# linwe2012/CourseComputationalPhotography

Measured on AMD Instinct MI355X. Metric: Gauss-Seidel pixel-updates/s on WxH 5-point Poisson grid, higher is better.
Workload: dtype f64

## Files before the change

### coursecomputationalphotography_amd/capi.py

```python
from __future__ import annotations

import atexit
import ctypes as C
import os
import sys
import weakref
from typing import Optional

import numpy as np

_HERE = os.path.dirname(os.path.abspath(__file__))
LIB_PATH = os.environ.get("CCP_GS_LIB") or os.path.join(_HERE, "lib", "libccp_gs.so")

CCP_OK = 0
GRID_DIRICHLET_MASK = 1
GRID_WEIGHTED = 2
MG_HIERARCHY_GALERKIN, MG_HIERARCHY_RESCALED = 0, 1
MG_HIERARCHIES = {"galerkin": MG_HIERARCHY_GALERKIN, "rescaled": MG_HIERARCHY_RESCALED}
ORDER_LEXICOGRAPHIC = 0
ORDER_MULTICOLOUR = 1
CLONE_IMPORT = 0
CLONE_MIXED = 1

ABI_SYMBOLS = (
    "ccp_status_string", "ccp_abi_version", "ccp_device_count",
    "ccp_csr_create", "ccp_csr_destroy", "ccp_csr_upload", "ccp_csr_upload_rows", "ccp_csr_rows_info", "ccp_csr_set_colouring", "ccp_csr_get_colouring", "ccp_csr_insert", "ccp_csr_insert_many", "ccp_csr_edit_stats", "ccp_csr_device_footprint", "ccp_csr_last_path", "ccp_csr_embed_region_host",
    "ccp_csr_gauss_seidel", "ccp_csr_conjugate_gradient", "ccp_csr_conjugate_gradient_jacobi", "ccp_csr_apply_to_vector", "ccp_csr_residual_norm2",
    "ccp_grid_create", "ccp_grid_destroy", "ccp_grid_get_layout", "ccp_grid_set_stream",
    "ccp_grid_synchronize", "ccp_grid_set_b_host", "ccp_grid_set_x_host", "ccp_grid_get_x_host",
    "ccp_grid_get_b_host", "ccp_grid_set_mask_host", "ccp_grid_fill_x", "ccp_grid_b_from_x", "ccp_grid_randomize_x",
    "ccp_grid_sweep", "ccp_grid_sweep_edges_first", "ccp_grid_stream_wait_edges", "ccp_grid_tune", "ccp_grid_set_fused", "ccp_grid_set_tiling", "ccp_grid_get_tiling", "ccp_grid_sweep_l1", "ccp_grid_halo_refreshed", "ccp_grid_gauss_seidel", "ccp_grid_gauss_seidel_lexicographic", "ccp_debug_lex_tickets", "ccp_grid_conjugate_gradient",
    "ccp_grid_mg_conjugate_gradient", "ccp_grid_mg_apply", "ccp_grid_mg_level",
    "ccp_grid_mg_set_hierarchy", "ccp_grid_mg_get_hierarchy",
    "ccp_grid_residual_norm2", "ccp_grid_abs_sum", "ccp_grid_assemble_rhs", "ccp_grid_assemble_from_images", "ccp_grid_store_u8",
    "ccp_grid_set_x_u8", "ccp_grid_assemble_region_rhs", "ccp_grid_assemble_clone", "ccp_grid_store_u8_composite",
    "ccp_grid_last_timing", "ccp_grid_region_begin", "ccp_grid_region_end",
    "ccp_grid_set_b_device", "ccp_grid_set_x_device", "ccp_grid_get_x_device", "ccp_grid_get_b_device",
    "ccp_grid_assemble_rhs_device", "ccp_grid_assemble_from_images_device", "ccp_grid_store_u8_device", "ccp_grid_set_x_u8_device",
    "ccp_grid_assemble_region_rhs_device", "ccp_grid_assemble_clone_device", "ccp_grid_store_u8_composite_device",
    "ccp_grid_set_weights_host", "ccp_grid_set_weights_device", "ccp_grid_assemble_weighted_rhs", "ccp_grid_assemble_weighted_rhs_device",
    "ccp_comm_probe", "ccp_comm_unique_id", "ccp_comm_create", "ccp_comm_destroy", "ccp_comm_info", "ccp_comm_all_reduce_sum", "ccp_comm_all_reduce_max",
    "ccp_grid_attach_comm", "ccp_grid_set_overlap", "ccp_grid_exchange_halos", "ccp_grid_sweep_rowblocked",
    "ccp_grid_gauss_seidel_rowblocked", "ccp_grid_conjugate_gradient_rowblocked", "ccp_grid_residual_norm2_global", "ccp_grid_comm_stats",
    "ccp_grid_mg_conjugate_gradient_rowblocked", "ccp_grid_mg_apply_rowblocked", "ccp_grid_mg_rowblock_info",
)


class CcpError(RuntimeError):
    def __init__(self, status: int, what: str):
        self.status = status
        super().__init__(f"{what}: status {status} ({status_string(status)})")


class Report(C.Structure):
    _fields_ = [("iterations", C.c_int32), ("converged", C.c_int32),
                ("last_l1_step", C.c_double), ("seconds", C.c_double)]


class GridDesc(C.Structure):
    _fields_ = [("width", C.c_int32), ("height", C.c_int32), ("channels", C.c_int32),
                ("row_begin", C.c_int32), ("row_count", C.c_int32), ("ghost", C.c_int32),
                ("device", C.c_int32), ("flags", C.c_int32)]


# ... 87 lines not shown
    L.ccp_csr_last_path.argtypes = [vp, C.POINTER(i32), C.POINTER(i32), C.POINTER(i32), C.POINTER(i64)]
    L.ccp_csr_edit_stats.argtypes = [vp] + [C.POINTER(i64)] * 5
    L.ccp_csr_device_footprint.argtypes = [vp] + [C.POINTER(i64)] * 2
    L.ccp_csr_gauss_seidel.argtypes = [vp, vp, vp, vp, dbl, i32, i32, i32, C.POINTER(Report)]
    L.ccp_csr_conjugate_gradient.argtypes = [vp, vp, vp, vp, dbl, i32, C.POINTER(Report)]
    L.ccp_csr_conjugate_gradient_jacobi.argtypes = [vp, vp, vp, dbl, i32, C.POINTER(Report)]
    L.ccp_grid_conjugate_gradient.argtypes = [vp, dbl, i32, C.POINTER(Report)]
    L.ccp_grid_mg_conjugate_gradient.argtypes = [vp, dbl, i32, i32, C.POINTER(Report)]
    L.ccp_grid_mg_apply.argtypes = [vp, i32]
    L.ccp_grid_mg_level.argtypes = [vp, i32] + [C.POINTER(i32)] * 3 + [vp] * 3
    L.ccp_grid_mg_set_hierarchy.argtypes = [vp, i32]
    L.ccp_grid_mg_get_hierarchy.argtypes = [vp, C.POINTER(i32)]
    L.ccp_csr_apply_to_vector.argtypes = [vp, vp, vp]
    L.ccp_csr_residual_norm2.argtypes = [vp, vp, vp, C.POINTER(dbl), C.POINTER(dbl)]
    L.ccp_grid_create.argtypes = [C.POINTER(GridDesc), C.POINTER(vp)]
    L.ccp_grid_destroy.argtypes = [vp]
    L.ccp_grid_get_layout.argtypes = [vp, C.POINTER(GridLayout)]
    L.ccp_grid_set_stream.argtypes = [vp, vp]
    L.ccp_grid_synchronize.argtypes = [vp]
    for name in ("ccp_grid_set_b_host", "ccp_grid_set_x_host", "ccp_grid_get_x_host", "ccp_grid_get_b_host"):
        getattr(L, name).argtypes = [vp, i32, vp, i32, i32]
    L.ccp_grid_set_mask_host.argtypes = [vp, vp, i64]
    L.ccp_grid_fill_x.argtypes = [vp, dbl]
    L.ccp_grid_b_from_x.argtypes = [vp]
    L.ccp_grid_randomize_x.argtypes = [vp, C.c_uint64, dbl, dbl]
    L.ccp_grid_sweep.argtypes = [vp, i32]
    L.ccp_grid_sweep_edges_first.argtypes = [vp, i32, i32]
    L.ccp_grid_stream_wait_edges.argtypes = [vp, vp]
    L.ccp_grid_sweep_l1.argtypes = [vp, vp]
    L.ccp_grid_tune.argtypes = [vp, i32, C.POINTER(i32), C.POINTER(i32), C.POINTER(C.c_float)]
    L.ccp_grid_set_fused.argtypes = [vp, i32]
    L.ccp_grid_set_tiling.argtypes = [vp, i32, i32]
    L.ccp_grid_get_tiling.argtypes = [vp, C.POINTER(i32), C.POINTER(i32), C.POINTER(i32)]
    L.ccp_grid_halo_refreshed.argtypes = [vp]
    L.ccp_grid_gauss_seidel.argtypes = [vp, dbl, i32, i32, C.POINTER(Report)]
    L.ccp_grid_gauss_seidel_lexicographic.argtypes = [vp, dbl, i32, i32, C.POINTER(Report)]
    L.ccp_grid_residual_norm2.argtypes = [vp, vp]
    L.ccp_grid_abs_sum.argtypes = [vp, vp]
    L.ccp_grid_assemble_rhs.argtypes = [vp, vp, vp, i64, vp]
    L.ccp_grid_assemble_from_images.argtypes = [vp, vp, i32, i64, vp, i64, i32]
    L.ccp_grid_store_u8.argtypes = [vp, vp, i64]
    L.ccp_grid_set_x_u8.argtypes = [vp, vp, i64]
    L.ccp_grid_assemble_region_rhs.argtypes = [vp, vp, vp, i64, vp, i64, i32]
    L.ccp_grid_assemble_clone.argtypes = [vp, vp, i64, vp, i64, i32, i32]
    L.ccp_grid_store_u8_composite.argtypes = [vp, vp, i64, vp, i64]
    da = C.POINTER(DeviceArray)
    for name in ("ccp_grid_set_b_device", "ccp_grid_set_x_device", "ccp_grid_get_x_device", "ccp_grid_get_b_device"):
        getattr(L, name).argtypes = [vp, da, i32, i32]
    L.ccp_grid_assemble_rhs_device.argtypes = [vp, da, da, vp]
    L.ccp_grid_assemble_from_images_device.argtypes = [vp, da, i32, da, i32]
    L.ccp_grid_store_u8_device.argtypes = [vp, da]
    L.ccp_grid_set_x_u8_device.argtypes = [vp, da]
    L.ccp_grid_assemble_region_rhs_device.argtypes = [vp, da, da, da, i32]
    L.ccp_grid_assemble_clone_device.argtypes = [vp, da, da, i32, i32]
    L.ccp_grid_store_u8_composite_device.argtypes = [vp, da, da]
    L.ccp_grid_set_weights_host.argtypes = [vp, vp, vp, vp, i64]
    L.ccp_grid_set_weights_device.argtypes = [vp, da, da, da]
    L.ccp_grid_assemble_weighted_rhs.argtypes = [vp, vp, vp, i64, vp, i64, i32]
    L.ccp_grid_assemble_weighted_rhs_device.argtypes = [vp, da, da, da, i32]
    L.ccp_grid_last_timing.argtypes = [vp, C.POINTER(C.c_float), C.POINTER(i32)]
    L.ccp_grid_region_begin.argtypes = [vp]
    L.ccp_grid_region_end.argtypes = [vp, C.POINTER(C.c_float), C.POINTER(i64), C.POINTER(i64)]
    L.ccp_comm_probe.argtypes = [i32]
    L.ccp_comm_unique_id.argtypes = [vp]
    L.ccp_comm_create.argtypes = [vp, i32, i32, i32, C.POINTER(vp)]
    L.ccp_comm_destroy.argtypes = [vp]
# ... 1 lines not shown
    L.ccp_comm_all_reduce_sum.argtypes = [vp, vp, i32]
    L.ccp_comm_all_reduce_max.argtypes = [vp, vp, i32]
    L.ccp_grid_attach_comm.argtypes = [vp, vp]
    L.ccp_grid_set_overlap.argtypes = [vp, i32]
    L.ccp_grid_exchange_halos.argtypes = [vp]
    L.ccp_grid_sweep_rowblocked.argtypes = [vp, i32]
    L.ccp_grid_gauss_seidel_rowblocked.argtypes = [vp, dbl, i32, i32, C.POINTER(Report)]
    L.ccp_grid_conjugate_gradient_rowblocked.argtypes = [vp, dbl, i32, C.POINTER(Report)]
    L.ccp_grid_mg_conjugate_gradient_rowblocked.argtypes = [vp, dbl, i32, i32, C.POINTER(Report)]
    L.ccp_grid_mg_apply_rowblocked.argtypes = [vp, i32]
    L.ccp_grid_mg_rowblock_info.argtypes = [vp] + [C.POINTER(i32)] * 4
    L.ccp_grid_residual_norm2_global.argtypes = [vp, vp]
    L.ccp_grid_comm_stats.argtypes = [vp, C.POINTER(i64), C.POINTER(i32), C.POINTER(i32), C.POINTER(i32)]
    _lib = L
    return L


def status_string(status: int) -> str:
    try:
        return load().ccp_status_string(status).decode()
    except Exception:
        return "?"


def check(status: int, what: str) -> None:
    if status != CCP_OK:
        raise CcpError(status, what)


def device_count() -> int:
    return int(load().ccp_device_count())


def _ptr(a: Optional[np.ndarray]):
    return None if a is None else a.ctypes.data_as(C.c_void_p)


def _f64(a) -> np.ndarray:
    return np.ascontiguousarray(a, dtype=np.float64)


def _i32(a) -> np.ndarray:
    return np.ascontiguousarray(a, dtype=np.int32)


def _no_overlap(shape, strides) -> bool:
    dims = sorted((s, e) for s, e in zip(strides, shape) if e > 1)
    span = 1
    for s, e in dims:
        if s < span:
            return False
        span = s * e
    return True


COMM_ID_BYTES = 128


def comm_probe(device: int = 0) -> None:
    _share_rccl_with_torch()
    check(load().ccp_comm_probe(device), "ccp_comm_probe")


def comm_unique_id() -> bytes:
    _share_rccl_with_torch()
    buf = (C.c_uint8 * COMM_ID_BYTES)()
# ... 681 lines not shown
```

### coursecomputationalphotography_amd/csrc/ccp_grid.hip

```cpp
#include "ccp_grid_kernels.hpp"
#include "ccp_grid_fused.hpp"
#include "ccp_grid_fused_wide.hpp"
#include "ccp_grid_lex.hpp"
#include "ccp_cg.hpp"
#include "ccp_grid_cg.hpp"
#include "ccp_grid_mg_view.hpp"
#include "ccp_grid_blend.hpp"
#include "ccp_grid_weighted.hpp"
#include "ccp_comm.hpp"

#include <algorithm>
#include <functional>
#include <cstring>
#include <chrono>
#include <vector>

using namespace ccp;

constexpr int kEdgeRing = 64;

struct ccp_grid {
    ccp_grid_desc desc{};
    Geom geom{};
    int ghost_top = 0, ghost_bottom = 0;
    bool shrink_top = false, shrink_bottom = false;
    int device = 0;
    hipStream_t stream = nullptr;
    hipStream_t stream2 = nullptr;
    hipEvent_t ev_main = nullptr, ev_side = nullptr;
    unsigned long long *edge_counter = nullptr;
    unsigned long long *edge_flag = nullptr;
    unsigned long long edge_epoch = 0;
    unsigned *edge_timeout = nullptr;
    unsigned long long edge_timeout_ticks = 200000000ull;
    int wait_mode = 0;
// ... 6 lines not shown
    hipEvent_t ev_comm = nullptr, ev_ready = nullptr;
    bool overlap = true;
    long exchanges = 0;
    DevBuf<double> x, b;
    DevBuf<double> cg_r, cg_p, cg_p2, cg_ap;
    DevBuf<CgState> cg_state;
    DevBuf<double> x_alt;
    bool allow_swap = false;
    bool masked = false;
    DevBuf<unsigned char> maskp, tile_live;
    DevBuf<int> tile_rows;
    DevBuf<unsigned char> mask_edge;
    bool mask_edge_known = false;
    int mask_border = -1;
    int live_T = -1, live_R = -1, live_lo = -1, live_hi = -1;
    long unknowns = 0;
    bool fuse = true;
    int multi = 0;
    DevBuf<unsigned> multi_words;
    bool xcd_swizzle = false;
    const char *trace_file = nullptr;
    DevBuf<unsigned long long> trace;
    bool short_edges = true;
    int side_rows_override = 0;
    int fuse_tmax = kFusedMaxT;
    int rows_per_chunk = 128;
    float tune_ms[kFusedMaxT + 1] = {0};
    int tune_rows[kFusedMaxT + 1] = {0};
    bool tuned = false;
    bool all_border = false;
    bool force_border = false;
    bool red_store_all = false;
    bool wide = true;
    DevBuf<double> partial;
    long partial_region = 0;
    DevBuf<double> small;
    DevBuf<unsigned> io_bad;
    DevBuf<double> sweep_sums;
    DevBuf<SolveState> state;
    DevBuf<int> redo_mask;
    DevBuf<double> lex_x, lex_b, lex_snap, lex_partial, lex_eps;
    DevBuf<unsigned> lex_progress, lex_ticket;
    DevBuf<double> lex_edges;
    int lex_mode = 3;
    int lex_tmax = 8;
    unsigned *lex_order_pin = nullptr;
    unsigned *lex_order_dev = nullptr;
    size_t lex_order_pin_cap = 0;
    size_t lex_order_count = 0;
    int lex_order_groups = 0, lex_order_strips = 0, lex_order_depth = 0;
    LexGeom lexg{};
    DevBuf<double> stage;
    long stage_rows = 0;
    int half_sweeps_since_refresh = 0;
    hipEvent_t ev0 = nullptr, ev1 = nullptr;
    hipEvent_t ev_r0 = nullptr, ev_r1 = nullptr;
    long region_launches = 0;
    long region_iterations = 0;
    float last_ms = 0.f;
    int last_launches = 0;
    bool timing_pending = false;
    int cpt = 2;
    int rows_per_block = 32;
    MgHierarchy *mg = nullptr;
    bool weighted = false;
    bool has_op = false;
// ... 243 lines not shown
            P.side_subs = std::max(P.side_subs, (std::max(P.first_rows, P.last_rows) + P.side_rows_edge - 1) / P.side_rows_edge);
    }
    const long n_border = (long)edge_chunks * (P.n_strips - edge_strips) + (long)P.n_chunks * edge_strips * P.side_subs;
    const bool any_plain = edge_chunks < P.n_chunks && edge_strips < P.n_strips;
    dim3 grid((unsigned)((P.n_strips + waves - 1) / waves), (unsigned)P.n_chunks, (unsigned)g->desc.channels);
    dim3 bgrid((unsigned)((n_border + waves - 1) / waves), 1, (unsigned)g->desc.channels);
    if (l1_blocks) {
        l1_blocks[0] = any_plain ? (long)grid.x * grid.y : 0;
        l1_blocks[1] = n_border ? (long)bgrid.x : 0;
    }
    if (l1 == 2 && T > kFusedMaxCheckedT) return CCP_ERR_BAD_ARG;
    const bool edge = want_edge && (P.first_edge || P.last_edge);
    P.edge_counter = g->edge_counter;
    P.edge_flag = g->edge_flag;
    P.edge_epoch = g->edge_epoch;
    P.edge_target = 0;
    if (edge) {
        long waves_expected = 0;
        for (int c = 0; c < P.n_chunks; c += std::max(1, P.n_chunks - 1)) {
            if (!fused_is_edge_chunk(P, c)) continue;
            int ra, rb;
            fused_chunk_rows(P, c, ra, rb);
            const int subs = std::min(P.side_subs, (rb - ra + P.side_rows_edge - 1) / P.side_rows_edge);
            waves_expected += (P.n_strips - edge_strips) + (long)edge_strips * subs;
        }
        P.edge_target = (unsigned long long)waves_expected * g->desc.channels;
        if (g->edge_epoch % kEdgeRing == 0) CCP_HIP(hipMemsetAsync(g->edge_counter, 0, sizeof(unsigned long long) * kEdgeRing, g->stream));
        P.edge_counter = g->edge_counter + (g->edge_epoch % kEdgeRing);
    }
    if (signalled) *signalled = edge;
    const bool wide = T == kWideT && g->wide && l1 == 0 && !edge && any_plain;
    const int wx0 = P.ns_left * U, wx1 = (P.n_strips - P.ns_right) * U;
    const int n_wide = wide ? (wx1 - wx0 + wide_useful_px(T) - 1) / wide_useful_px(T) : 0;
    const dim3 wgrid((unsigned)((n_wide + kWideWaves - 1) / kWideWaves), (unsigned)(P.n_chunks - edge_chunks), (unsigned)g->desc.channels);
    const dim3 pgrid = wide ? wgrid : grid;
    const size_t trace_plain = (size_t)pgrid.x * pgrid.y * pgrid.z * waves * 4, trace_border = (size_t)bgrid.x * bgrid.z * waves * 4;
    unsigned long long *trace_p = nullptr, *trace_b = nullptr;
    if (g->trace_file) {
        if (g->trace.n < trace_plain + trace_border) CCP_TRY(g->trace.alloc(trace_plain + trace_border));
        CCP_HIP(hipMemsetAsync(g->trace.p, 0, (trace_plain + trace_border) * sizeof(unsigned long long), g->stream));
        trace_p = g->trace.p;
        trace_b = g->trace.p + trace_plain;
    }
    P.trace = trace_b;
    constexpr int TC = T <= kFusedMaxCheckedT ? T : 1;
    hipStream_t bstream = g->stream2;
    if (n_border) {
        CCP_HIP(hipEventRecord(g->ev_main, g->stream));
        CCP_HIP(hipStreamWaitEvent(bstream, g->ev_main, 0));
    }
    if (n_border && edge) {
        hipLaunchKernelGGL((k_fused_border<T, 0, kFusedUnroll, true>), bgrid, dim3(kBlock), 0, bstream, P, g->force_border ? 1 : 0);
    }
    if (any_plain) {
        P.trace = trace_p;
        if (l1 == 2) hipLaunchKernelGGL((k_fused_sweep<TC, 2, kFusedUnroll>), grid, dim3(kBlock), 0, g->stream, P);
        else if (l1 == 1) hipLaunchKernelGGL((k_fused_sweep<T, 1, kFusedUnroll>), grid, dim3(kBlock), 0, g->stream, P);
        else if (edge) hipLaunchKernelGGL((k_fused_sweep<T, 0, kFusedUnroll, true>), grid, dim3(kBlock), 0, g->stream, P);
        else if (wide && !store_red) hipLaunchKernelGGL((k_fused_sweep_wide<kWideT, false>), wgrid, dim3(kBlock), 0, g->stream, P, wx0, wx1, n_wide);
        else if (wide) hipLaunchKernelGGL((k_fused_sweep_wide<kWideT, true>), wgrid, dim3(kBlock), 0, g->stream, P, wx0, wx1, n_wide);
        else if (!store_red) hipLaunchKernelGGL((k_fused_sweep<T, 0, kFusedUnroll, false, false>), grid, dim3(kBlock), 0, g->stream, P);
        else hipLaunchKernelGGL((k_fused_sweep<T, 0, kFusedUnroll>), grid, dim3(kBlock), 0, g->stream, P);
    }
    if (n_border) {
        const int fb = g->force_border ? 1 : 0;
        P.trace = trace_b;
        if (l1 == 2) hipLaunchKernelGGL((k_fused_border<TC, 2, kFusedUnroll>), bgrid, dim3(kBlock), 0, bstream, P, fb);
        else if (l1 == 1) hipLaunchKernelGGL((k_fused_border<T, 1, kFusedUnroll>), bgrid, dim3(kBlock), 0, bstream, P, fb);
        else if (!edge) hipLaunchKernelGGL((k_fused_border<T, 0, kFusedUnroll>), bgrid, dim3(kBlock), 0, bstream, P, fb);
        CCP_HIP(hipEventRecord(g->ev_side, bstream));
        CCP_HIP(hipStreamWaitEvent(g->stream, g->ev_side, 0));
    }
    CCP_HIP(hipGetLastError());
    if (g->trace_file) {
        CCP_HIP(hipStreamSynchronize(g->stream));
        std::vector<unsigned long long> host(trace_plain + trace_border);
        CCP_HIP(hipMemcpy(host.data(), g->trace.p, host.size() * sizeof(unsigned long long), hipMemcpyDeviceToHost));
        if (FILE *f = fopen(g->trace_file, "ab")) {
            const unsigned long long head[8] = {0x43435054524143ull, (unsigned long long)T, pgrid.x, pgrid.y, pgrid.z, bgrid.x, (unsigned long long)host.size(),
                                                (unsigned long long)P.rows_per_chunk};
            fwrite(head, sizeof(head), 1, f);
            fwrite(host.data(), sizeof(unsigned long long), host.size(), f);
            fclose(f);
        }
    }
    g->last_launches++;
    g->region_launches++;
    g->region_iterations += T;
    return CCP_OK;
}

template <int T>
int launch_fused_multi_t(ccp_grid *g, int n_passes, const double *xin, double *xout, const int *st_lo, const int *st_hi, int red_skip = 0)
{
    if (n_passes < 2 || n_passes > kMultiMaxPasses || g->trace_file) return CCP_ERR_UNSUPPORTED;
    if (g->masked && T > kMaskedMaxT) return CCP_ERR_UNSUPPORTED;
    FusedMultiParams M{};
    FusedParams &P = M.P;
    P.xin = xin;
    P.xout = xout;
    P.b = g->b.p;
    P.g = g->geom;
    P.st_lo = st_lo[0];
    P.st_hi = st_hi[0];
    P.rows_per_chunk = (g->tuned && g->tune_rows[T] > 0) ? g->tune_rows[T] : g->rows_per_chunk;
    const int U = fused_useful_px(T);
    P.n_strips = (g->geom.W + U - 1) / U;
    P.partial = g->partial.p;
    P.partial_border = g->partial.p + g->partial_region;
    P.active = nullptr;
    P.xcd_swizzle = 0;
    P.mask = g->maskp.p;
    P.trace = nullptr;
// ... 291 lines not shown
        if (TO_DEVICE) {
            CCP_HIP(hipMemcpyAsync(g->stage.p, host, bytes, hipMemcpyHostToDevice, g->stream));
            hipLaunchKernelGGL((k_convert<true>), grid, dim3(kBlock), 0, g->stream, dev_base, g->stage.p,
                               g->geom, channel, l_first, W);
            CCP_HIP(hipGetLastError());
        } else {
            hipLaunchKernelGGL((k_convert<false>), grid, dim3(kBlock), 0, g->stream, dev_base, g->stage.p,
                               g->geom, channel, l_first, W);
            CCP_HIP(hipGetLastError());
            CCP_HIP(hipMemcpyAsync(host, g->stage.p, bytes, hipMemcpyDeviceToHost, g->stream));
        }
        CCP_HIP(hipStreamSynchronize(g->stream));
        done += chunk;
    }
    return edge_timeout_status(g);
}

}

extern "C" {

int ccp_grid_create(const ccp_grid_desc *d, ccp_grid **out)
try {
    if (!d || !out) return CCP_ERR_BAD_ARG;
    *out = nullptr;
    if (d->width < 1 || d->height < 1 || d->channels < 1 || d->channels > kMaxChannels) return CCP_ERR_BAD_ARG;
    if (d->row_begin < 0 || d->row_count < 1 || d->row_begin + d->row_count > d->height || d->ghost < 0)
        return CCP_ERR_BAD_ARG;
    if ((long)d->width * d->height > 0x7fffffffL) return CCP_ERR_BAD_ARG;
    if ((d->flags & CCP_GRID_WEIGHTED) &&
        ((d->flags & CCP_GRID_DIRICHLET_MASK) || d->ghost != 0 || d->row_begin != 0 || d->row_count != d->height))
        return CCP_ERR_UNSUPPORTED;
    CCP_TRY(select_device(d->device));
    ccp_grid *g = new (std::nothrow) ccp_grid();
    if (!g) return CCP_ERR_ALLOC;
    g->desc = *d;
    g->device = d->device;
    g->ghost_top = d->row_begin > 0 ? std::min(d->ghost, d->row_begin) : 0;
    g->ghost_bottom = (d->row_begin + d->row_count < d->height) ? std::min(d->ghost, d->height - d->row_begin - d->row_count) : 0;
    Geom &geo = g->geom;
    geo.W = d->width;
    geo.H = d->height;
    geo.y0 = d->row_begin - g->ghost_top;
    g->shrink_top = geo.y0 > 0;
    g->shrink_bottom = d->row_begin + d->row_count + g->ghost_bottom < d->height;
    geo.local_rows = g->ghost_top + d->row_count + g->ghost_bottom;
    geo.own_lo = g->ghost_top;
    geo.own_hi = g->ghost_top + d->row_count;
    geo.pitch = (((long)d->width + 1) / 2 + 15) / 16 * 16;
    geo.ch_stride = (long)geo.local_rows * 2 * geo.pitch;
    g->cpt = 2;
    if (const char *e = getenv("CCP_GS_FUSE")) g->fuse = atoi(e) != 0;
    if (const char *e = getenv("CCP_GS_SHORT_EDGES")) g->short_edges = atoi(e) != 0;
    if (const char *e = getenv("CCP_GS_XCD")) g->xcd_swizzle = atoi(e) != 0;
    if (const char *e = getenv("CCP_GS_MULTI")) g->multi = atoi(e);
    if (const char *e = getenv("CCP_GS_TRACE_FILE")) g->trace_file = e[0] ? e : nullptr;
    if (const char *e = getenv("CCP_GS_SIDE_ROWS")) g->side_rows_override = atoi(e);
    if (const char *e = getenv("CCP_GS_LEX_MODE"))
        g->lex_mode = strcmp(e, "planes") == 0 ? 0 : 3;
    if (const char *e = getenv("CCP_GS_TMAX")) g->fuse_tmax = std::max(1, std::min(kFusedMaxT, atoi(e)));
    if (const char *e = getenv("CCP_GS_ALL_BORDER")) g->all_border = atoi(e) != 0;
    if (const char *e = getenv("CCP_GS_FORCE_BORDER")) g->force_border = atoi(e) != 0;
    if (const char *e = getenv("CCP_GS_RED_STORE")) g->red_store_all = atoi(e) != 0;
    if (const char *e = getenv("CCP_GS_WIDE")) g->wide = atoi(e) != 0;
    if (const char *e = getenv("CCP_GS_CHUNK")) g->rows_per_chunk = std::max(1, atoi(e));
    choose_tiling(g);
    g->masked = (d->flags & CCP_GRID_DIRICHLET_MASK) != 0;
    if (g->masked) {
        g->fuse_tmax = std::min(g->fuse_tmax, kMaskedMaxT);
        if (!getenv("CCP_GS_CHUNK")) g->rows_per_chunk = 160;
    }

    const size_t elems = (size_t)geo.ch_stride * d->channels;
    int st = g->x.alloc(elems);
    if (st == CCP_OK && g->masked) {
        st = g->maskp.alloc((size_t)geo.ch_stride);
        if (st == CCP_OK && hipMemset(g->maskp.p, 0, (size_t)geo.ch_stride) != hipSuccess) st = CCP_ERR_HIP;
        if (st == CCP_OK) st = g->mask_edge.alloc(2 * (size_t)d->width);
        if (st == CCP_OK && hipMemset(g->mask_edge.p, 0, 2 * (size_t)d->width) != hipSuccess) st = CCP_ERR_HIP;
    }
    if (st == CCP_OK) st = g->b.alloc(elems);
    g->weighted = (d->flags & CCP_GRID_WEIGHTED) != 0;
    if (st == CCP_OK && g->weighted) {
        st = g->wop.alloc(4 * (size_t)geo.ch_stride);
        if (st == CCP_OK && hipMemset(g->wop.p, 0, 4 * sizeof(double) * (size_t)geo.ch_stride) != hipSuccess) st = CCP_ERR_HIP;
        if (st == CCP_OK) st = g->wpart.alloc(4 * (size_t)d->channels * kWeightedApplyBlocks);
    }
    const size_t part = (size_t)((geo.pitch + 2L * kBlock - 1) / (2L * kBlock)) * geo.local_rows * d->channels * 2 * 2 + 64;
    g->partial_region = (long)(part / 2);
    if (st == CCP_OK) st = g->partial.alloc(part);
    if (st == CCP_OK) st = g->small.alloc(4 * kMaxChannels);
    if (st == CCP_OK) st = g->io_bad.alloc(1);
    if (st == CCP_OK) st = g->state.alloc(1);
    g->stage_rows = std::max<long>(1, std::min<long>(geo.local_rows, (8L << 20) / d->width));
    if (st == CCP_OK) st = g->stage.alloc((size_t)g->stage_rows * d->width);
    if (st == CCP_OK && (hipEventCreate(&g->ev0) != hipSuccess || hipEventCreate(&g->ev1) != hipSuccess)) st = CCP_ERR_HIP;
    if (st == CCP_OK && (hipStreamCreateWithFlags(&g->stream2, hipStreamNonBlocking) != hipSuccess ||
// ... 441 lines not shown
        }
    }
    if (chosen_t) *chosen_t = best_t;
    if (chosen_rows_per_chunk) *chosen_rows_per_chunk = best_r;
    if (ms_per_iteration) *ms_per_iteration = best;
    return CCP_OK;
} CCP_ABI_CATCH

int ccp_grid_set_fused(ccp_grid *g, int32_t on)
try {
    CCP_TRY(not_weighted(g));
    if (!g) return CCP_ERR_BAD_ARG;
    g->fuse = on != 0;
    return CCP_OK;
} CCP_ABI_CATCH

int ccp_grid_set_tiling(ccp_grid *g, int32_t max_t, int32_t rows_per_chunk)
try {
    CCP_TRY(not_weighted(g));
    if (!g || max_t < 1 || rows_per_chunk < 2) return CCP_ERR_BAD_ARG;
    g->fuse_tmax = std::min<int>(max_t, kFusedMaxT);
    g->rows_per_chunk = rows_per_chunk + (rows_per_chunk & 1);
    g->tuned = false;
    return CCP_OK;
} CCP_ABI_CATCH

int ccp_grid_get_tiling(ccp_grid *g, int32_t *max_t, int32_t *rows_per_chunk, int32_t *tuned)
try {
    if (!g) return CCP_ERR_BAD_ARG;
    const int T = g->fuse_tmax;
    if (max_t) *max_t = T;
    if (rows_per_chunk) *rows_per_chunk = (g->tuned && g->tune_rows[T] > 0) ? g->tune_rows[T] : g->rows_per_chunk;
    if (tuned) *tuned = g->tuned ? 1 : 0;
    return CCP_OK;
} CCP_ABI_CATCH

int ccp_grid_sweep_l1(ccp_grid *g, double *l1_per_channel)
try {
    CCP_TRY(not_weighted(g));
    CCP_TRY(bind(g));
    if (!l1_per_channel) return CCP_ERR_BAD_ARG;
    const int C = g->desc.channels;
    CCP_TRY(begin_timing(g));
    long blocks[2] = {0, 0};
    CCP_TRY(one_iteration(g, true, nullptr, blocks));
    hipLaunchKernelGGL(k_check, dim3((unsigned)C), dim3(kBlock), 0, g->stream, g->partial.p, blocks[0],
                       g->partial.p + g->partial_region, blocks[1], 0.0, 0, static_cast<SolveState *>(nullptr), g->small.p);
    CCP_HIP(hipGetLastError());
    CCP_TRY(end_timing(g));
    CCP_HIP(hipMemcpyAsync(l1_per_channel, g->small.p, sizeof(double) * C, hipMemcpyDeviceToHost, g->stream));
    CCP_HIP(hipStreamSynchronize(g->stream));
    return CCP_OK;
} CCP_ABI_CATCH

int ccp_grid_gauss_seidel(ccp_grid *g, double epsilon, int32_t max_iteration, int32_t check_every, ccp_gs_report *report)
try {
    CCP_TRY(not_weighted(g));
    CCP_TRY(bind(g));
    if (g->ghost_top || g->ghost_bottom) return CCP_ERR_STATE;
    if (check_every < 0) return CCP_ERR_BAD_ARG;
    const int C = g->desc.channels;
    SolveState host{};
    for (int ch = 0; ch < C; ++ch) {
        host.active[ch] = 1;
        host.last_eps[ch] = 10.0;
    }
// ... 1751 lines not shown
```

### coursecomputationalphotography_amd/csrc/ccp_grid_fused.hpp

```cpp
#pragma once

#include "ccp_grid_kernels.hpp"

namespace ccp {

#ifndef CCP_FUSED_MAX_T
#define CCP_FUSED_MAX_T 8
#endif
constexpr int kFusedMaxT = CCP_FUSED_MAX_T;
constexpr int kFusedMaxCheckedT = 8;
#ifndef CCP_FUSED_UNROLL
#define CCP_FUSED_UNROLL 2
#endif
constexpr int kFusedUnroll = CCP_FUSED_UNROLL;
#ifndef CCP_FUSED_LAND
#define CCP_FUSED_LAND 2
#endif
constexpr int kFusedLand = CCP_FUSED_LAND;
constexpr int kStripLanes = kWave;

__host__ __device__ constexpr int fused_halo_px(int T) { return 2 * T; }
__host__ __device__ constexpr int fused_useful_px(int T) { return 2 * kStripLanes - 4 * T; }

__device__ __forceinline__ double lane_prev(double v)
{
    int lo = __double2loint(v), hi = __double2hiint(v);
    lo = __builtin_amdgcn_update_dpp(0, lo, 0x138, 0xf, 0xf, true);
    hi = __builtin_amdgcn_update_dpp(0, hi, 0x138, 0xf, 0xf, true);
    return __hiloint2double(hi, lo);
}
__device__ __forceinline__ double lane_next(double v)
{
    int lo = __double2loint(v), hi = __double2hiint(v);
    lo = __builtin_amdgcn_update_dpp(0, lo, 0x130, 0xf, 0xf, true);
    hi = __builtin_amdgcn_update_dpp(0, hi, 0x130, 0xf, 0xf, true);
    return __hiloint2double(hi, lo);
}

struct FusedParams {
    const double *__restrict__ xin;
    double *__restrict__ xout;
    const double *__restrict__ b;
    Geom g;
    int st_lo, st_hi;
    int rows_per_chunk;
    int first_rows, last_rows;
    int n_strips;
    double *__restrict__ partial;
    const int *__restrict__ active;
    int n_chunks;
    int nb_top, nb_bot, ns_left, ns_right;
    int side_rows, side_subs;
    int side_rows_edge;
    double *__restrict__ partial_border;
    const unsigned char *__restrict__ mask;
    int first_edge, last_edge;
    int xcd_swizzle;
    unsigned long long *__restrict__ trace;
    unsigned long long *__restrict__ edge_counter;
    unsigned long long *__restrict__ edge_flag;
    unsigned long long edge_target, edge_epoch;
};

__host__ __device__ __forceinline__ int fused_chunk_of(const FusedParams &P, int y)
{
    const int n_e = P.first_edge + P.last_edge;
    if (y < n_e) return (P.first_edge && y == 0) ? 0 : P.n_chunks - 1;
    return y - n_e + P.first_edge;
}

__host__ __device__ __forceinline__ bool fused_is_edge_chunk(const FusedParams &P, int chunk)
{
    return (P.first_edge && chunk == 0) || (P.last_edge && chunk == P.n_chunks - 1);
}

__device__ __forceinline__ void fused_signal_edge(const FusedParams &P)
{
    __builtin_amdgcn_fence(__ATOMIC_RELEASE, "agent");
    if ((threadIdx.x & (kWave - 1)) == 0) {
        const unsigned long long old = __hip_atomic_fetch_add(P.edge_counter, 1ull, __ATOMIC_RELAXED, __HIP_MEMORY_SCOPE_AGENT);
        if (old + 1 == P.edge_target)
            __hip_atomic_store(P.edge_flag, P.edge_epoch, __ATOMIC_RELEASE, __HIP_MEMORY_SCOPE_SYSTEM);
    }
}

__device__ __forceinline__ void fused_tile_coords(const FusedParams &P, unsigned &bx, unsigned &by, unsigned &bz)
{
    bx = blockIdx.x;
    by = blockIdx.y;
    bz = blockIdx.z;
// ... 683 lines not shown
```

### coursecomputationalphotography_amd/csrc/ccp_grid_fused_wide.hpp

```cpp
#pragma once

#include "ccp_grid_fused.hpp"

namespace ccp {

constexpr int kWideT = 8;
constexpr int kWideRing = 20;
constexpr int kWideWaves = kBlock / kWave;
__host__ __device__ constexpr int wide_useful_px(int T) { return 4 * kStripLanes - 4 * T; }

typedef unsigned int u32x4 __attribute__((ext_vector_type(4)));
typedef double d2 __attribute__((ext_vector_type(2)));

__device__ __forceinline__ d2 buf_load2(__amdgpu_buffer_rsrc_t rs, unsigned voff)
{
    return __builtin_bit_cast(d2, __builtin_amdgcn_raw_buffer_load_b128(rs, (int)voff, 0, 0));
}
__device__ __forceinline__ void buf_store2(d2 v, __amdgpu_buffer_rsrc_t rs, unsigned voff)
{
    __builtin_amdgcn_raw_buffer_store_b128(__builtin_bit_cast(u32x4, v), rs, (int)voff, 0, 0);
}

struct WideCtx {
    const double *__restrict__ xin;
// ... 121 lines not shown
    cx.st_k = col_store ? cx.ld_k : kLaneOut;
    cx.ra = ra; cx.rb = rb;
    cx.m0 = max(ra - HS, 0);
    cx.m1 = min(rb + HS, g.local_rows);
    const int base = cx.m0 - ((g.y0 + cx.m0) & 1);
    const int f_end = rb - 1 + HS;

    d2 wr[NT], wk[NT];
    d2 la[G][4], lb[G][4];
#pragma unroll
    for (int s = 0; s < NT; ++s) wr[s] = wk[s] = d2{0.0, 0.0};
#pragma unroll
    for (int s = 0; s < kWideRing; ++s) {
        cx.ring[s * 2 * kWave] = d2{0.0, 0.0};
        cx.ring[s * 2 * kWave + kWave] = d2{0.0, 0.0};
    }
#pragma unroll
    for (int i = 0; i < G; ++i) wide_load_row(cx, g, base + i, la[i]);
#pragma unroll
    for (int i = 0; i < G; ++i) wide_load_row(cx, g, base + G + i, lb[i]);
#pragma unroll
    for (int i = 0; i < G; ++i) wide_place(wr, wk, cx, Win::slot(i, 0), i, la[i]);
    for (int fb = base; fb <= f_end; fb += kWideRing) wide_turn<T, STORE_RED, NT, 0>(wr, wk, cx, g, fb, la, lb);
}

template <int T, bool STORE_RED>
__global__ void __launch_bounds__(kBlock, 2)
k_fused_sweep_wide(FusedParams P, int wx0, int wx1, int n_wide)
{
    __shared__ d2 ring[kWideWaves][kWideRing * 2 * kWave];
    const int wave = __builtin_amdgcn_readfirstlane(threadIdx.x / kWave);
    unsigned bx, by, bz;
    fused_tile_coords(P, bx, by, bz);
    const int sw = (int)bx * kWideWaves + wave;
    const int ch = (int)bz;
    const int chunk = P.nb_top + (int)by;
    int ra, rb;
    fused_chunk_rows(P, chunk, ra, rb);
    const bool run = (P.active == nullptr) || (P.active[ch] != 0);
    if (run && sw < n_wide && ra < rb) {
        const Geom &g = P.g;
        const long off = (long)ch * g.ch_stride;
        unsigned long long t0 = 0;
        fused_trace_begin(P, t0);
        fused_wave_wide<T, STORE_RED>(P.xin + off, P.xout + off, P.b + off, g, wx0, wx1, sw, ra, rb, ring[wave]);
        fused_trace_end(P, t0, (((long)blockIdx.z * gridDim.y + blockIdx.y) * gridDim.x + blockIdx.x) * kWideWaves + wave, chunk, sw, ch, 3);
    }
}

}
```

### include/ccp_gs.h

```cpp
#ifndef CCP_GS_H
#define CCP_GS_H

#include <stddef.h>
#include <stdint.h>

#ifdef __cplusplus
extern "C" {
#endif

#define CCP_GS_ABI_VERSION 6

typedef enum ccp_status {
    CCP_OK = 0,
    CCP_ERR_BAD_ARG = 1,
    CCP_ERR_NO_DEVICE = 2,
    CCP_ERR_HIP = 3,
    CCP_ERR_ALLOC = 4,
    CCP_ERR_STATE = 5,
    CCP_ERR_UNSUPPORTED = 6,
    CCP_ERR_RCCL = 7
} ccp_status;

typedef enum ccp_ordering {
    CCP_ORDER_LEXICOGRAPHIC = 0,
// ... 79 lines not shown
    void   *x_dev;
    void   *b_dev;
    int64_t pitch;
    int32_t local_rows;
    int32_t ghost_top;
    int32_t ghost_bottom;
    int32_t channels;
} ccp_grid_layout;

int ccp_grid_create(const ccp_grid_desc *desc, ccp_grid **out);
int ccp_grid_destroy(ccp_grid *g);
int ccp_grid_get_layout(ccp_grid *g, ccp_grid_layout *out);
int ccp_grid_set_stream(ccp_grid *g, void *hip_stream);
int ccp_grid_synchronize(ccp_grid *g);

int ccp_grid_set_b_host(ccp_grid *g, int32_t channel, const double *rows, int32_t first_row, int32_t n_rows);
int ccp_grid_set_x_host(ccp_grid *g, int32_t channel, const double *rows, int32_t first_row, int32_t n_rows);
int ccp_grid_get_x_host(ccp_grid *g, int32_t channel, double *rows, int32_t first_row, int32_t n_rows);
int ccp_grid_get_b_host(ccp_grid *g, int32_t channel, double *rows, int32_t first_row, int32_t n_rows);
int ccp_grid_set_mask_host(ccp_grid *g, const uint8_t *mask, int64_t row_stride_bytes);
int ccp_grid_fill_x(ccp_grid *g, double value);
int ccp_grid_b_from_x(ccp_grid *g);
int ccp_grid_randomize_x(ccp_grid *g, uint64_t seed, double lo, double hi);

int ccp_grid_sweep(ccp_grid *g, int32_t iterations);

int ccp_grid_sweep_edges_first(ccp_grid *g, int32_t iterations, int32_t edge_rows);
int ccp_grid_stream_wait_edges(ccp_grid *g, void *hip_stream);
int ccp_grid_tune(ccp_grid *g, int32_t max_t, int32_t *chosen_t, int32_t *chosen_rows_per_chunk,
                  float *ms_per_iteration);
int ccp_grid_set_fused(ccp_grid *g, int32_t on);
int ccp_grid_set_tiling(ccp_grid *g, int32_t max_t, int32_t rows_per_chunk);
int ccp_grid_get_tiling(ccp_grid *g, int32_t *max_t, int32_t *rows_per_chunk, int32_t *tuned);
int ccp_grid_sweep_l1(ccp_grid *g, double *l1_per_channel);
int ccp_grid_halo_refreshed(ccp_grid *g);

int ccp_grid_gauss_seidel(ccp_grid *g, double epsilon, int32_t max_iteration,
                          int32_t check_every, ccp_gs_report *report);

int ccp_grid_gauss_seidel_lexicographic(ccp_grid *g, double epsilon, int32_t max_iteration,
                                        int32_t check_every, ccp_gs_report *report);

int ccp_debug_lex_tickets(int32_t width, int32_t depth, int32_t groups, uint32_t *order, int64_t capacity, int32_t *strips,
                          int64_t *count);

int ccp_grid_conjugate_gradient(ccp_grid *g, double epsilon, int32_t max_iteration, ccp_gs_report *report);

int ccp_grid_mg_conjugate_gradient(ccp_grid *g, double epsilon, int32_t max_iteration, int32_t smoothing_sweeps,
                                   ccp_gs_report *report);
int ccp_grid_mg_apply(ccp_grid *g, int32_t smoothing_sweeps);
int ccp_grid_mg_level(ccp_grid *g, int32_t level, int32_t *n_levels, int32_t *width, int32_t *height, double *diag,
                      double *w_east, double *w_south);

#define CCP_MG_HIERARCHY_GALERKIN 0
#define CCP_MG_HIERARCHY_RESCALED 1
int ccp_grid_mg_set_hierarchy(ccp_grid *g, int32_t kind);
int ccp_grid_mg_get_hierarchy(ccp_grid *g, int32_t *kind);

#define CCP_COMM_ID_BYTES 128
typedef struct ccp_comm ccp_comm;
int ccp_comm_probe(int32_t device);
int ccp_comm_unique_id(uint8_t *id_out );
int ccp_comm_create(const uint8_t *id , int32_t rank, int32_t world, int32_t device, ccp_comm **out);
int ccp_comm_destroy(ccp_comm *c);
int ccp_comm_info(ccp_comm *c, int32_t *rank, int32_t *world, int32_t *device, int32_t *rccl_version);
int ccp_comm_all_reduce_sum(ccp_comm *c, double *values, int32_t count);
// ... 80 lines not shown
```

Measured before the change: 2124 billion.

## Flatten wide kernel launch and add occupancy-aware row segment planner

Replaces the 3D wide-kernel grid (strip, chunk, channel) with a flat 1D wave index decoded into channel, row segment and strip. Adds a cost-model planner that picks the segment height to balance wave count against CU slots and per-segment march overhead, exposed via an API and env var. By default segmentation still follows the existing chunk size, so the planner is opt-in. The flat decode adds a few integer divisions per wave and assumes uniform segment heights.

```diff
diff --git a/coursecomputationalphotography_amd/capi.py b/coursecomputationalphotography_amd/capi.py
--- a/coursecomputationalphotography_amd/capi.py
+++ b/coursecomputationalphotography_amd/capi.py
@@ -29,7 +29,7 @@
     "ccp_grid_create", "ccp_grid_destroy", "ccp_grid_get_layout", "ccp_grid_set_stream",
     "ccp_grid_synchronize", "ccp_grid_set_b_host", "ccp_grid_set_x_host", "ccp_grid_get_x_host",
     "ccp_grid_get_b_host", "ccp_grid_set_mask_host", "ccp_grid_fill_x", "ccp_grid_b_from_x", "ccp_grid_randomize_x",
-    "ccp_grid_sweep", "ccp_grid_sweep_edges_first", "ccp_grid_stream_wait_edges", "ccp_grid_tune", "ccp_grid_set_fused", "ccp_grid_set_tiling", "ccp_grid_get_tiling", "ccp_grid_sweep_l1", "ccp_grid_halo_refreshed", "ccp_grid_gauss_seidel", "ccp_grid_gauss_seidel_lexicographic", "ccp_debug_lex_tickets", "ccp_grid_conjugate_gradient",
+    "ccp_grid_sweep", "ccp_grid_sweep_edges_first", "ccp_grid_stream_wait_edges", "ccp_grid_tune", "ccp_grid_set_fused", "ccp_grid_set_tiling", "ccp_grid_get_tiling", "ccp_wide_plan", "ccp_grid_sweep_l1", "ccp_grid_halo_refreshed", "ccp_grid_gauss_seidel", "ccp_grid_gauss_seidel_lexicographic", "ccp_debug_lex_tickets", "ccp_grid_conjugate_gradient",
     "ccp_grid_mg_conjugate_gradient", "ccp_grid_mg_apply", "ccp_grid_mg_level",
     "ccp_grid_mg_set_hierarchy", "ccp_grid_mg_get_hierarchy",
     "ccp_grid_residual_norm2", "ccp_grid_abs_sum", "ccp_grid_assemble_rhs", "ccp_grid_assemble_from_images", "ccp_grid_store_u8",
@@ -183,6 +183,7 @@
     L.ccp_grid_set_fused.argtypes = [vp, i32]
     L.ccp_grid_set_tiling.argtypes = [vp, i32, i32]
     L.ccp_grid_get_tiling.argtypes = [vp, C.POINTER(i32), C.POINTER(i32), C.POINTER(i32)]
+    L.ccp_wide_plan.argtypes = [i32, i32, i32, i32, C.POINTER(i32), C.POINTER(i32)]
     L.ccp_grid_halo_refreshed.argtypes = [vp]
     L.ccp_grid_gauss_seidel.argtypes = [vp, dbl, i32, i32, C.POINTER(Report)]
     L.ccp_grid_gauss_seidel_lexicographic.argtypes = [vp, dbl, i32, i32, C.POINTER(Report)]
@@ -250,6 +251,12 @@
     return int(load().ccp_device_count())
 
 
+def wide_plan(rows: int, n_wide: int, channels: int, cus: int):
+    seg, n = C.c_int32(), C.c_int32()
+    check(load().ccp_wide_plan(rows, n_wide, channels, cus, C.byref(seg), C.byref(n)), "ccp_wide_plan")
+    return seg.value, n.value
+
+
 def _ptr(a: Optional[np.ndarray]):
     return None if a is None else a.ctypes.data_as(C.c_void_p)
 
diff --git a/coursecomputationalphotography_amd/csrc/ccp_grid.hip b/coursecomputationalphotography_amd/csrc/ccp_grid.hip
--- a/coursecomputationalphotography_amd/csrc/ccp_grid.hip
+++ b/coursecomputationalphotography_amd/csrc/ccp_grid.hip
@@ -1,6 +1,7 @@
 #include "ccp_grid_kernels.hpp"
 #include "ccp_grid_fused.hpp"
 #include "ccp_grid_fused_wide.hpp"
+#include "ccp_wide_plan.hpp"
 #include "ccp_grid_lex.hpp"
 #include "ccp_cg.hpp"
 #include "ccp_grid_cg.hpp"
@@ -73,6 +74,8 @@
     bool force_border = false;
     bool red_store_all = false;
     bool wide = true;
+    int wide_segs = kWideSegsDefault;
+    int cus = 0;
     DevBuf<double> partial;
     long partial_region = 0;
     DevBuf<double> small;
@@ -382,7 +385,18 @@
     const bool wide = T == kWideT && g->wide && l1 == 0 && !edge && any_plain;
     const int wx0 = P.ns_left * U, wx1 = (P.n_strips - P.ns_right) * U;
     const int n_wide = wide ? (wx1 - wx0 + wide_useful_px(T) - 1) / wide_useful_px(T) : 0;
-    const dim3 wgrid((unsigned)((n_wide + kWideWaves - 1) / kWideWaves), (unsigned)(P.n_chunks - edge_chunks), (unsigned)g->desc.channels);
+    P.wide_lo = P.wide_hi = P.wide_seg_rows = P.wide_segs = P.wide_waves = 0;
+    if (wide) {
+        int r0, r1;
+        fused_chunk_rows(P, P.nb_top, P.wide_lo, r1);
+        fused_chunk_rows(P, P.n_chunks - P.nb_bot - 1, r0, P.wide_hi);
+        const WidePlan plan = g->wide_segs == 0 ? WidePlan{P.rows_per_chunk, P.n_chunks - edge_chunks}
+                                                : wide_plan(P.wide_hi - P.wide_lo, n_wide, g->desc.channels, g->cus, std::max(0, g->wide_segs));
+        P.wide_seg_rows = plan.seg_rows;
+        P.wide_segs = plan.n_segs;
+        P.wide_waves = n_wide * plan.n_segs * g->desc.channels;
+    }
+    const dim3 wgrid((unsigned)((P.wide_waves + kWideWaves - 1) / kWideWaves), 1, 1);
     const dim3 pgrid = wide ? wgrid : grid;
     const size_t trace_plain = (size_t)pgrid.x * pgrid.y * pgrid.z * waves * 4, trace_border = (size_t)bgrid.x * bgrid.z * waves * 4;
     unsigned long long *trace_p = nullptr, *trace_b = nullptr;
@@ -428,7 +442,7 @@
         CCP_HIP(hipMemcpy(host.data(), g->trace.p, host.size() * sizeof(unsigned long long), hipMemcpyDeviceToHost));
         if (FILE *f = fopen(g->trace_file, "ab")) {
             const unsigned long long head[8] = {0x43435054524143ull, (unsigned long long)T, pgrid.x, pgrid.y, pgrid.z, bgrid.x, (unsigned long long)host.size(),
-                                                (unsigned long long)P.rows_per_chunk};
+                                                (unsigned long long)P.rows_per_chunk | ((unsigned long long)P.wide_seg_rows << 32)};
             fwrite(head, sizeof(head), 1, f);
             fwrite(host.data(), sizeof(unsigned long long), host.size(), f);
             fclose(f);
@@ -786,8 +800,11 @@
         ((d->flags & CCP_GRID_DIRICHLET_MASK) || d->ghost != 0 || d->row_begin != 0 || d->row_count != d->height))
         return CCP_ERR_UNSUPPORTED;
     CCP_TRY(select_device(d->device));
+    int cus = 0;
+    CCP_HIP(hipDeviceGetAttribute(&cus, hipDeviceAttributeMultiprocessorCount, d->device));
     ccp_grid *g = new (std::nothrow) ccp_grid();
     if (!g) return CCP_ERR_ALLOC;
+    g->cus = std::max(1, cus);
     g->desc = *d;
     g->device = d->device;
     g->ghost_top = d->row_begin > 0 ? std::min(d->ghost, d->row_begin) : 0;
@@ -817,6 +834,7 @@
     if (const char *e = getenv("CCP_GS_FORCE_BORDER")) g->force_border = atoi(e) != 0;
     if (const char *e = getenv("CCP_GS_RED_STORE")) g->red_store_all = atoi(e) != 0;
     if (const char *e = getenv("CCP_GS_WIDE")) g->wide = atoi(e) != 0;
+    if (const char *e = getenv("CCP_GS_WIDE_SEGS")) g->wide_segs = std::max(-1, atoi(e));
     if (const char *e = getenv("CCP_GS_CHUNK")) g->rows_per_chunk = std::max(1, atoi(e));
     choose_tiling(g);
     g->masked = (d->flags & CCP_GRID_DIRICHLET_MASK) != 0;
@@ -1324,6 +1342,16 @@
     if (max_t) *max_t = T;
     if (rows_per_chunk) *rows_per_chunk = (g->tuned && g->tune_rows[T] > 0) ? g->tune_rows[T] : g->rows_per_chunk;
     if (tuned) *tuned = g->tuned ? 1 : 0;
+    return CCP_OK;
+} CCP_ABI_CATCH
+
+int ccp_wide_plan(int32_t rows, int32_t n_wide, int32_t channels, int32_t cus, int32_t *segment_rows, int32_t *segments)
+try {
+    if (rows < 1 || n_wide < 1 || channels < 1 || cus < 1 || !segment_rows || !segments) return CCP_ERR_BAD_ARG;
+    static_assert(kWidePlanT == kWideT && kWidePlanRing == kWideRing && kWidePlanWaves == kWideWaves, "the planner models the wide kernel");
+    const WidePlan plan = wide_plan(rows, n_wide, channels, cus);
+    *segment_rows = plan.seg_rows;
+    *segments = plan.n_segs;
     return CCP_OK;
 } CCP_ABI_CATCH
 
diff --git a/coursecomputationalphotography_amd/csrc/ccp_grid_fused.hpp b/coursecomputationalphotography_amd/csrc/ccp_grid_fused.hpp
--- a/coursecomputationalphotography_amd/csrc/ccp_grid_fused.hpp
+++ b/coursecomputationalphotography_amd/csrc/ccp_grid_fused.hpp
@@ -56,6 +56,7 @@
     const unsigned char *__restrict__ mask;
     int first_edge, last_edge;
     int xcd_swizzle;
+    int wide_lo, wide_hi, wide_seg_rows, wide_segs, wide_waves;
     unsigned long long *__restrict__ trace;
     unsigned long long *__restrict__ edge_counter;
     unsigned long long *__restrict__ edge_flag;
diff --git a/coursecomputationalphotography_amd/csrc/ccp_grid_fused_wide.hpp b/coursecomputationalphotography_amd/csrc/ccp_grid_fused_wide.hpp
--- a/coursecomputationalphotography_amd/csrc/ccp_grid_fused_wide.hpp
+++ b/coursecomputationalphotography_amd/csrc/ccp_grid_fused_wide.hpp
@@ -177,19 +177,22 @@
     const int wave = __builtin_amdgcn_readfirstlane(threadIdx.x / kWave);
     unsigned bx, by, bz;
     fused_tile_coords(P, bx, by, bz);
-    const int sw = (int)bx * kWideWaves + wave;
-    const int ch = (int)bz;
-    const int chunk = P.nb_top + (int)by;
-    int ra, rb;
-    fused_chunk_rows(P, chunk, ra, rb);
+    const int w = (int)bx * kWideWaves + wave;
+    if (w >= P.wide_waves) return;
+    const int per_ch = n_wide * P.wide_segs;
+    const int ch = w / per_ch;
+    const int seg = (w - ch * per_ch) / n_wide;
+    const int sw = w - ch * per_ch - seg * n_wide;
+    const int ra = P.wide_lo + seg * P.wide_seg_rows;
+    const int rb = min(ra + P.wide_seg_rows, P.wide_hi);
     const bool run = (P.active == nullptr) || (P.active[ch] != 0);
-    if (run && sw < n_wide && ra < rb) {
+    if (run && ra < rb) {
         const Geom &g = P.g;
         const long off = (long)ch * g.ch_stride;
         unsigned long long t0 = 0;
         fused_trace_begin(P, t0);
         fused_wave_wide<T, STORE_RED>(P.xin + off, P.xout + off, P.b + off, g, wx0, wx1, sw, ra, rb, ring[wave]);
-        fused_trace_end(P, t0, (((long)blockIdx.z * gridDim.y + blockIdx.y) * gridDim.x + blockIdx.x) * kWideWaves + wave, chunk, sw, ch, 3);
+        fused_trace_end(P, t0, (long)blockIdx.x * kWideWaves + wave, seg, sw, ch, 3);
     }
 }
 
diff --git a/coursecomputationalphotography_amd/csrc/ccp_wide_plan.hpp b/coursecomputationalphotography_amd/csrc/ccp_wide_plan.hpp
--- /dev/null
+++ b/coursecomputationalphotography_amd/csrc/ccp_wide_plan.hpp
@@ -0,0 +1,62 @@
+#pragma once
+
+namespace ccp {
+
+struct WidePlan {
+    int seg_rows;
+    int n_segs;
+};
+
+constexpr int kWidePlanT = 8;
+constexpr int kWidePlanRing = 20;
+constexpr int kWidePlanWaves = 4;
+constexpr int kWidePlanMinRows = 2 * kWidePlanT + 16;
+constexpr int kWidePlanReserve = 8;
+
+#ifndef CCP_WIDE_SEGS_DEFAULT
+#define CCP_WIDE_SEGS_DEFAULT 0
+#endif
+constexpr int kWideSegsDefault = CCP_WIDE_SEGS_DEFAULT;
+
+inline int wide_plan_cus(int cus) { return cus - cus / kWidePlanReserve; }
+
+inline int wide_plan_march(int seg_rows)
+{
+    return (seg_rows + 4 * kWidePlanT + kWidePlanRing - 1) / kWidePlanRing * kWidePlanRing;
+}
+
+inline int wide_plan_seg_rows(int rows, int count)
+{
+    int s = (rows + count - 1) / count;
+    s += s & 1;
+    return s < kWidePlanMinRows ? kWidePlanMinRows : s;
+}
+
+inline long wide_plan_cost(int seg_rows, int n_segs, int n_wide, int channels, int cus)
+{
+    const long waves = (long)n_wide * n_segs * channels, slots = (long)kWidePlanWaves * wide_plan_cus(cus);
+    return (waves + slots - 1) / slots * wide_plan_march(seg_rows);
+}
+
+inline WidePlan wide_plan(int rows, int n_wide, int channels, int cus, int force_segs = 0)
+{
+    WidePlan best{kWidePlanMinRows, 1};
+    if (rows < 1 || n_wide < 1 || channels < 1) return best;
+    if (cus < 1) cus = 1;
+    const int max_count = (rows + kWidePlanMinRows - 1) / kWidePlanMinRows;
+    const int lo = force_segs > 0 ? (force_segs < max_count ? force_segs : max_count) : 1;
+    const int hi = force_segs > 0 ? lo : max_count;
+    long best_cost = -1;
+    for (int count = lo; count <= hi; ++count) {
+        const int s = wide_plan_seg_rows(rows, count);
+        const int n = (rows + s - 1) / s;
+        const long c = wide_plan_cost(s, n, n_wide, channels, cus);
+        if (best_cost < 0 || c < best_cost || (c == best_cost && s < best.seg_rows)) {
+            best_cost = c;
+            best = WidePlan{s, n};
+        }
+    }
+    return best;
+}
+
+}
diff --git a/include/ccp_gs.h b/include/ccp_gs.h
--- a/include/ccp_gs.h
+++ b/include/ccp_gs.h
@@ -135,6 +135,7 @@
 int ccp_grid_set_fused(ccp_grid *g, int32_t on);
 int ccp_grid_set_tiling(ccp_grid *g, int32_t max_t, int32_t rows_per_chunk);
 int ccp_grid_get_tiling(ccp_grid *g, int32_t *max_t, int32_t *rows_per_chunk, int32_t *tuned);
+int ccp_wide_plan(int32_t rows, int32_t n_wide, int32_t channels, int32_t cus, int32_t *segment_rows, int32_t *segments);
 int ccp_grid_sweep_l1(ccp_grid *g, double *l1_per_channel);
 int ccp_grid_halo_refreshed(ccp_grid *g);
 
```

After: 2095 billion. 0.986x the previous value.
